# gusanagy/Hybrid-Diffusion-Underwater-Atmopheric-Image-Enhancement

Measured on AMD Instinct MI355X. Metric: denoising-steps/sec (256x256, T=1000), higher is better.
Workload: dtype f32 (tensors and accumulation fp32; every operand of the attention contractions as 2xfp16 pieces -- scores: a balance per product term, four terms at d_head 16 / three at d_head 32; P.V: three terms -- and of the 3x3 convs behind GroupNorm likewise (other 3x3 convs: 3xbf16 pieces), on the 16-bit MFM

## Files before the change

hybrid-diffusion-underwater-atmopheric-image-enhancement_amd/_capi.py:

```python
from __future__ import annotations

import ctypes as C
import os
import subprocess

_HERE = os.path.dirname(os.path.abspath(__file__))
LIB_PATH = os.environ.get("HDIFF_LIB", os.path.join(_HERE, "libhdiff.so"))
CSRC = os.path.join(_HERE, "csrc")
MAX_TAPS = 25

_lib = None


class LinearJob(C.Structure):
    _fields_ = [("w0", C.c_void_p), ("b0", C.c_void_p), ("w1", C.c_void_p), ("b1", C.c_void_p), ("y", C.c_void_p),
                ("n", C.c_int), ("first", C.c_int)]


class DdpmLoopDesc(C.Structure):
    _fields_ = [
        ("x", C.c_void_p), ("eps_c", C.c_void_p), ("eps_u", C.c_void_p), ("noise", C.c_void_p), ("x_next", C.c_void_p),
        ("coeff1", C.c_void_p), ("coeff2", C.c_void_p), ("sigma", C.c_void_p), ("step_ptr", C.c_void_p), ("T", C.c_int),
        ("w", C.c_double), ("seed", C.c_uint64), ("nan_flag", C.c_void_p), ("n", C.c_int64),
        ("x_dup0", C.c_void_p), ("x_dup1", C.c_void_p), ("t_next", C.c_void_p), ("t_count", C.c_int),
# ... 52 lines not shown
    ]


class WgradDesc(C.Structure):
    _fields_ = [
        ("x0", C.c_void_p), ("x1", C.c_void_p), ("C0", C.c_int), ("C1", C.c_int),
        ("B", C.c_int), ("H", C.c_int), ("W", C.c_int),
        ("gn_scale", C.c_void_p), ("gn_shift", C.c_void_p), ("dy", C.c_void_p),
        ("Cout", C.c_int), ("CinPad", C.c_int), ("CoutPad", C.c_int), ("OH", C.c_int), ("OW", C.c_int),
        ("VH", C.c_int), ("VW", C.c_int), ("in_stride", C.c_int),
        ("out_sy", C.c_int), ("out_oy", C.c_int), ("out_sx", C.c_int), ("out_ox", C.c_int),
        ("ntaps", C.c_int), ("tap_dy", C.c_int * MAX_TAPS), ("tap_dx", C.c_int * MAX_TAPS),
    ]


_PROTOS = {
    "hdiff_abi_version": (C.c_int, []),
    "hdiff_last_error": (C.c_char_p, []),
    "hdiff_device_count": (C.c_int, []),
    "hdiff_pack_conv_weight_x3": (C.c_int, [C.c_void_p, C.c_void_p, C.c_int, C.c_int, C.c_int, C.c_int, C.c_void_p]),
    "hdiff_pack_conv_weight_x3_taps": (C.c_int, [C.c_void_p, C.c_void_p, C.c_int, C.c_int, C.c_int, C.c_int, C.c_int, C.c_int,
                                                 C.POINTER(C.c_int), C.POINTER(C.c_int), C.c_int, C.c_void_p]),
    "hdiff_pack_conv_weight_h2_words": (C.c_int, [C.c_int, C.c_int, C.c_int, C.POINTER(C.c_int64)]),
    "hdiff_pack_conv_weight_h2": (C.c_int, [C.c_void_p, C.c_void_p, C.c_int, C.c_int, C.c_int, C.c_void_p]),
    "hdiff_gn_act_scale": (C.c_int, [C.c_void_p, C.c_void_p, C.c_int, C.c_int64, C.c_float, C.c_void_p, C.c_void_p]),
    "hdiff_set_contraction_mode": (C.c_int, [C.c_int]),
    "hdiff_get_contraction_mode": (C.c_int, []),
    "hdiff_pack_conv_weight": (C.c_int, [C.c_void_p, C.c_void_p, C.c_int, C.c_int, C.c_int, C.c_int, C.c_int, C.c_int,
                                         C.POINTER(C.c_int), C.POINTER(C.c_int), C.c_int, C.c_int, C.c_int, C.c_void_p]),
    "hdiff_conv2d_fwd": (C.c_int, [C.POINTER(ConvDesc), C.c_void_p]),
    "hdiff_conv2d_fwd_dropout": (C.c_int, [C.POINTER(ConvDesc), C.c_void_p, C.c_float, C.c_void_p]),
    "hdiff_conv2d_fwd_range": (C.c_int, [C.POINTER(ConvDesc), C.POINTER(ConvRange), C.c_void_p]),
    "hdiff_range_words_zero": (C.c_int, [C.c_void_p, C.c_int, C.c_void_p]),
    "hdiff_conv2d_fwd_route": (C.c_int, [C.POINTER(ConvDesc), C.POINTER(ConvRange), C.c_int, C.POINTER(C.c_int), C.POINTER(C.c_int)]),
    "hdiff_pack_conv_weight_h2_taps_words": (C.c_int, [C.c_int, C.c_int, C.c_int, C.c_int, C.POINTER(C.c_int64)]),
    "hdiff_pack_conv_weight_h2_taps": (C.c_int, [C.c_void_p, C.c_void_p, C.c_int, C.c_int, C.c_int, C.c_int, C.c_int, C.c_int,
                                                 C.POINTER(C.c_int), C.POINTER(C.c_int), C.c_int, C.c_void_p]),
    "hdiff_pack_conv_weight_h2_s2_words": (C.c_int, [C.c_int, C.c_int, C.c_int, C.POINTER(C.c_int64)]),
    "hdiff_pack_conv_weight_h2_s2": (C.c_int, [C.c_void_p, C.c_void_p, C.c_int, C.c_int, C.c_int, C.c_int, C.c_void_p]),
    "hdiff_conv2d_fwd_workspace": (C.c_int, [C.POINTER(ConvDesc), C.POINTER(C.c_int64)]),
    "hdiff_gn_stats": (C.c_int, [C.c_void_p, C.c_void_p, C.c_int, C.c_int, C.c_int, C.c_int, C.c_int, C.c_int, C.c_void_p,
                                 C.c_void_p]),
    "hdiff_gn_finalize": (C.c_int, [C.c_void_p, C.c_int, C.c_int, C.c_int, C.c_int, C.c_void_p, C.c_void_p, C.c_float,
                                    C.c_void_p, C.c_void_p, C.c_void_p, C.c_void_p, C.c_void_p]),
    "hdiff_gn_scale_shift": (C.c_int, [C.c_void_p, C.c_void_p, C.c_int, C.c_int, C.c_int, C.c_int, C.c_int, C.c_int, C.c_void_p,
                                       C.c_void_p, C.c_void_p, C.c_float, C.c_void_p, C.c_void_p, C.c_void_p]),
    "hdiff_gn_swish_apply": (C.c_int, [C.c_void_p, C.c_void_p, C.c_void_p, C.c_void_p, C.c_int, C.c_int, C.c_int,
                                       C.c_void_p]),
    "hdiff_mha_flash_fwd": (C.c_int, [C.c_void_p, C.c_void_p, C.c_void_p, C.c_int, C.c_int, C.c_int, C.c_int, C.c_void_p]),
    "hdiff_mha_flash_fwd_workspace": (C.c_int, [C.c_int, C.c_int, C.c_int, C.c_int, C.POINTER(C.c_int64)]),
    "hdiff_mha_flash_fwd_ws": (C.c_int, [C.c_void_p, C.c_void_p, C.c_void_p, C.c_int, C.c_int, C.c_int, C.c_int, C.c_void_p,
                                         C.c_int64, C.c_void_p]),
    "hdiff_mha_flash_fwd_route": (C.c_int, [C.c_int, C.c_int, C.c_int, C.c_int, C.c_int, C.c_int64] + [C.POINTER(C.c_int)] * 3),
    "hdiff_mha_wide_fwd": (C.c_int, [C.c_void_p, C.c_void_p, C.c_int, C.c_int, C.c_int, C.c_void_p]),
    "hdiff_mha_wide_bwd": (C.c_int, [C.c_void_p, C.c_void_p, C.c_void_p, C.c_void_p, C.c_int, C.c_int, C.c_int, C.c_void_p]),
    "hdiff_gn_affine_bwd": (C.c_int, [C.c_void_p, C.c_int, C.c_int, C.c_int, C.c_int, C.c_void_p, C.c_void_p, C.c_void_p, C.c_void_p,
                                      C.c_void_p, C.c_void_p, C.c_void_p, C.c_void_p, C.c_void_p, C.c_void_p]),
    "hdiff_gn_affine_apply": (C.c_int, [C.c_void_p, C.c_void_p, C.c_void_p, C.c_void_p, C.c_int, C.c_int, C.c_int,
                                        C.c_void_p]),
    "hdiff_mha_flash_bwd_workspace": (C.c_int, [C.c_int, C.c_int, C.c_int, C.c_int, C.POINTER(C.c_int64)]),
    "hdiff_mha_flash_bwd": (C.c_int, [C.c_void_p, C.c_void_p, C.c_void_p, C.c_void_p, C.c_void_p, C.c_void_p, C.c_void_p,
                                      C.c_int, C.c_int, C.c_int, C.c_int, C.c_void_p]),
    "hdiff_mha_flash_bwd_route": (C.c_int, [C.c_int, C.c_int, C.c_int, C.c_int] + [C.POINTER(C.c_int)] * 4),
    "hdiff_conv2d_wgrad_workspace": (C.c_int, [C.POINTER(WgradDesc), C.POINTER(C.c_int), C.POINTER(C.c_int64)]),
    "hdiff_conv2d_wgrad": (C.c_int, [C.POINTER(WgradDesc), C.c_void_p, C.c_int, C.c_void_p]),
    "hdiff_conv2d_wgrad_dropout": (C.c_int, [C.POINTER(WgradDesc), C.c_void_p, C.c_float, C.c_void_p, C.c_int, C.c_void_p]),
    "hdiff_conv2d_wgrad_route": (C.c_int, [C.POINTER(WgradDesc), C.c_int, C.POINTER(C.c_int)]),
    "hdiff_conv_wgrad_unpack": (C.c_int, [C.c_void_p, C.c_int, C.c_void_p, C.c_int, C.c_int, C.c_int, C.c_int, C.c_int, C.c_int,
                                          C.POINTER(C.c_int), C.POINTER(C.c_int), C.c_int, C.c_int, C.c_int, C.c_void_p]),
    "hdiff_gn_swish_bwd": (C.c_int, [C.c_void_p, C.c_void_p, C.c_int, C.c_int, C.c_int, C.c_int, C.c_int, C.c_void_p, C.c_void_p,
                                     C.c_void_p, C.c_void_p, C.c_void_p, C.c_void_p, C.c_void_p, C.c_void_p, C.c_void_p,
                                     C.c_void_p, C.c_void_p]),
    "hdiff_gn_swish_dropout_bwd": (C.c_int, [C.c_void_p, C.c_int, C.c_int, C.c_int, C.c_int, C.c_void_p, C.c_void_p, C.c_float,
                                             C.c_void_p, C.c_void_p, C.c_void_p, C.c_void_p, C.c_void_p, C.c_void_p, C.c_void_p,
                                             C.c_void_p, C.c_void_p]),
    "hdiff_bias_addvec_grad": (C.c_int, [C.c_void_p, C.c_int, C.c_int, C.c_int, C.c_void_p, C.c_void_p, C.c_void_p]),
    "hdiff_linear_rows_bwd": (C.c_int, [C.c_void_p, C.c_void_p, C.c_int, C.c_void_p, C.c_void_p, C.c_void_p, C.c_void_p,
                                        C.c_void_p, C.c_int, C.c_int, C.c_int, C.c_int, C.c_int, C.c_int, C.c_void_p]),
    "hdiff_sq_err_bwd": (C.c_int, [C.c_void_p, C.c_void_p, C.c_void_p, C.c_void_p, C.c_int64, C.c_void_p]),
    "hdiff_dropout_mask": (C.c_int, [C.c_void_p, C.c_int64, C.c_float, C.c_uint64, C.c_uint64, C.c_void_p]),
    "hdiff_dropout_keep_bits": (C.c_int, [C.c_void_p, C.c_int64, C.c_float, C.c_uint64, C.c_uint64, C.c_void_p]),
    "hdiff_mul": (C.c_int, [C.c_void_p, C.c_void_p, C.c_void_p, C.c_int64, C.c_void_p]),
    "hdiff_linear_rows": (C.c_int, [C.c_void_p, C.c_void_p, C.c_int, C.c_void_p, C.c_void_p, C.c_void_p, C.c_int, C.c_int,
                                    C.c_int, C.c_int, C.c_int, C.c_void_p]),
    "hdiff_linear_rows_multi": (C.c_int, [C.c_void_p, C.c_void_p, C.c_void_p, C.c_int, C.c_int, C.c_int, C.c_int, C.c_void_p]),
    "hdiff_q_sample": (C.c_int, [C.c_void_p, C.c_void_p, C.c_void_p, C.c_void_p, C.c_void_p, C.c_void_p, C.c_int, C.c_int,
                                 C.c_int, C.c_void_p]),
    "hdiff_sq_err": (C.c_int, [C.c_void_p, C.c_void_p, C.c_void_p, C.c_int64, C.c_void_p]),
    "hdiff_ddpm_step": (C.c_int, [C.c_void_p, C.c_void_p, C.c_void_p, C.c_void_p, C.c_void_p, C.c_void_p, C.c_void_p,
                                  C.c_void_p, C.c_void_p, C.c_int, C.c_double, C.c_uint64, C.c_void_p, C.c_int64, C.c_void_p]),
    "hdiff_ddpm_step_loop": (C.c_int, [C.c_void_p, C.c_void_p]),
    "hdiff_cfg_ddim_step": (C.c_int, [C.c_void_p, C.c_void_p, C.c_void_p, C.c_void_p, C.c_void_p, C.c_void_p, C.c_void_p, C.c_int,
                                      C.c_double, C.c_int, C.c_uint64, C.c_void_p, C.c_int64, C.c_void_p]),
    "hdiff_cfg_ddim_step_loop": (C.c_int, [C.c_void_p, C.c_void_p]),
    "hdiff_cfg_dpmpp_step": (C.c_int, [C.c_void_p, C.c_void_p, C.c_void_p, C.c_void_p, C.c_void_p, C.c_void_p, C.c_void_p, C.c_int,
                                       C.c_double, C.c_int, C.c_void_p, C.c_int64, C.c_void_p]),
    "hdiff_cfg_dpmpp_step_loop": (C.c_int, [C.c_void_p, C.c_void_p]),
    "hdiff_fill_t": (C.c_int, [C.c_void_p, C.c_void_p, C.c_int, C.c_void_p]),
    "hdiff_step_decrement": (C.c_int, [C.c_void_p, C.c_void_p]),
    "hdiff_ddim_step": (C.c_int, [C.c_void_p, C.c_void_p, C.c_void_p, C.c_void_p, C.c_void_p, C.c_int, C.c_void_p, C.c_int64,
                                  C.c_void_p]),
    "hdiff_fill_from_table": (C.c_int, [C.c_void_p, C.c_void_p, C.c_void_p, C.c_int, C.c_int, C.c_void_p]),
    "hdiff_tile_gather": (C.c_int, [C.c_void_p] * 4 + [C.c_int] * 10 + [C.c_void_p]),
    "hdiff_tile_ddim_step": (C.c_int, [C.c_void_p] * 12 + [C.c_int, C.c_void_p] + [C.c_int] * 8 + [C.c_void_p]),
    "hdiff_dpmpp_step": (C.c_int, [C.c_void_p] * 6 + [C.c_int, C.c_int, C.c_void_p, C.c_int64, C.c_void_p]),
    "hdiff_tile_dpmpp_step": (C.c_int, [C.c_void_p] * 13 + [C.c_int, C.c_int, C.c_void_p] + [C.c_int] * 8 + [C.c_void_p]),
# ... 146 lines not shown
```

hybrid-diffusion-underwater-atmopheric-image-enhancement_amd/csrc/attention.hip:

```cpp
#include <stdlib.h>

#include <type_traits>

#include "common.h"
#include "device.h"

using namespace hdiff;

namespace {

constexpr int KT = 64;
constexpr int KROW = KT + 4;
constexpr int ATT_THREADS = 256;
constexpr float RESCALE_LIMIT = 1.8446744e19f;

__device__ __forceinline__ f32x2 pk_add(f32x2 a, f32x2 b) {
  f32x2 r;
  asm("v_pk_add_f32 %0, %1, %2" : "=v"(r) : "v"(a), "v"(b));
  return r;
}

template <int D, int NQ>
__global__ __launch_bounds__(ATT_THREADS) void mha_flash_fwd_kernel(const float* __restrict__ qkv, float* __restrict__ out,
                                                                    float* __restrict__ lse2, int C, int L, float qscale, int check) {
// ... 384 lines not shown
  stage_load(0);
  stage_store(0);
  __syncthreads();
  stage_load(ntiles > 1 ? 1 : 0);
  do_tile(std::true_type{}, 0);
  stage_store(1);
  __syncthreads();
  auto step = [&](int t, auto buf_tag) {
    constexpr int buf = decltype(buf_tag)::value;
    stage_load((t + 1 < ntiles) ? t + 1 : t);
    do_tile(std::false_type{}, buf);
    stage_store(buf ^ 1);
    __syncthreads();
  };
  int t = 1;
  for (; t + 1 < ntiles; t += 2) {
    step(t, std::integral_constant<int, 1>{});
    step(t + 1, std::integral_constant<int, 0>{});
  }
  if (t < ntiles) step(t, std::integral_constant<int, 1>{});
  rowsum(NQ - 1);

  float* obase = out + ((size_t)b * C + (size_t)head * D) * L;
#pragma unroll
  for (int qt = 0; qt < NQ; ++qt) {
    float lt = l_run[qt].x + l_run[qt].y;
    lt += __shfl_xor(lt, 16, 64);
    lt += __shfl_xor(lt, 32, 64);
    const bool bad = !(lt < OVERFLOW_LIMIT);
    const float inv = bad ? __builtin_nanf("") : 1.0f / lt;
    const int q = qblk0 + qt * 16 + i16;
    if (lse2 != nullptr && q < L && g == 0)
      lse2[((size_t)b * gridDim.y + head) * L + q] = bad ? __builtin_nanf("") : __builtin_amdgcn_logf(lt) - negm4[qt][0];
    if (q < L) {
#pragma unroll
      for (int mt = 0; mt < MT; ++mt)
#pragma unroll
        for (int r = 0; r < 4; ++r) {
          const int d = mt * 16 + 4 * g + r;
          if (d < D) obase[(size_t)d * L + q] = O[mt][qt][r] * inv;
        }
    }
  }
}

template <int D, int NQ>
void launch_v(const float* qkv, float* o, float* lse2, int B, int C, int heads, int L, float qscale, int check,
              hipStream_t stream) {
  dim3 grid(cdiv(L, 64 * NQ), heads, B);
  hipLaunchKernelGGL((mha_flash_fwd_kernel<D, NQ>), grid, dim3(ATT_THREADS), 0, stream, qkv, o, lse2, C, L, qscale, check);
}

struct MhaFwdRoute { int route, nq, check; };
MhaFwdRoute mha_fwd_route(int B, int C, int heads, int L, bool want_lse, int64_t ws_bytes, int mode) {
  const int D = C / heads;
  if (D >= 48 || L < 512) return {HDIFF_MHA_FWD_ROUTE_RUNNING_MAX, 1, 0};
  if (mode != HDIFF_CONTRACT_F32) {
    const int64_t need = mha_fwd_x3p_workspace(B, C, heads, L);
    const bool ws_ok = need != 0 && ws_bytes >= need;
    if (mode == HDIFF_CONTRACT_F16 && !want_lse && ws_ok) return {HDIFF_MHA_FWD_ROUTE_F16_SINGLE, 4, 1};
    if (ws_ok && D == 16) return {HDIFF_MHA_FWD_ROUTE_H2_PAIRS, 4, 1};
    if (ws_ok && D == 32) return {HDIFF_MHA_FWD_ROUTE_X3P_PAIRS, 4, 1};
    if (L % KT == 0 && (D == 16 || D == 32)) return {HDIFF_MHA_FWD_ROUTE_X3_TRIPLES, 4, 1};
  }
  if (L % KT == 0) return {HDIFF_MHA_FWD_ROUTE_FAST_F32, 4, 1};
  return {HDIFF_MHA_FWD_ROUTE_RUNNING_MAX, 4, 0};
}

template <int D>
void launch_d(const float* qkv, float* o, float* lse2, int B, int C, int heads, int L, void* ws, const MhaFwdRoute& rt,
              hipStream_t stream) {
  const float qscale = 1.4426950408889634f / sqrtf((float)D);
  static const bool skip_check = getenv("HDIFF_NO_CHECK_PASS") != nullptr;
  const bool tail = !skip_check || rt.route == HDIFF_MHA_FWD_ROUTE_RUNNING_MAX || rt.route == HDIFF_MHA_FWD_ROUTE_FAST_F32;
  if constexpr (D < 48) {
    switch (rt.route) {
      case HDIFF_MHA_FWD_ROUTE_F16_SINGLE: launch_mha_fwd_f16(qkv, o, B, C, heads, L, qscale, ws, stream); break;
      case HDIFF_MHA_FWD_ROUTE_H2_PAIRS: launch_mha_fwd_h2(qkv, o, lse2, B, C, heads, L, qscale, ws, stream); break;
      case HDIFF_MHA_FWD_ROUTE_X3P_PAIRS: launch_mha_fwd_x3p(qkv, o, lse2, B, C, heads, L, qscale, ws, stream); break;
      case HDIFF_MHA_FWD_ROUTE_X3_TRIPLES: launch_mha_fwd_x3(qkv, o, lse2, B, C, heads, L, qscale, stream); break;
      case HDIFF_MHA_FWD_ROUTE_FAST_F32:
        hipLaunchKernelGGL((mha_flash_fwd_fast_kernel<D, 4>), dim3(cdiv(L, 256), heads, B), dim3(ATT_THREADS), 0, stream, qkv, o, lse2, C, L, qscale);
        break;
      default: break;
    }
    if (tail && rt.nq == 4) launch_v<D, 4>(qkv, o, lse2, B, C, heads, L, qscale, rt.check, stream);
  }
  if (tail && rt.nq == 1) launch_v<D, 1>(qkv, o, lse2, B, C, heads, L, qscale, rt.check, stream);
}

}

static int mha_fwd_check_shape(int B, int C, int heads, int L) {
  HDIFF_CHECK_ARG(B > 0 && L > 0 && heads > 0 && C % heads == 0, "mha_flash_fwd: bad sizes B=%d C=%d heads=%d L=%d", B, C,
                  heads, L);
  HDIFF_CHECK_ARG(mha_head_dim_ok(C / heads), "mha_flash_fwd: head dim %d not in {4, 8, 12, 16, 24, 32, 48, 64}", C / heads);
  return HDIFF_OK;
}

static int mha_flash_fwd_any(const float* qkv, float* o, float* lse2, int B, int C, int heads, int L, void* ws,
                             int64_t ws_bytes, hipStream_t s) {
  HDIFF_CHECK_ARG(qkv && o, "mha_flash_fwd: null pointer");
  const int rc = mha_fwd_check_shape(B, C, heads, L);
  if (rc != HDIFF_OK) return rc;
  const MhaFwdRoute rt = mha_fwd_route(B, C, heads, L, lse2 != nullptr, ws_bytes, contraction_mode());
  (void)hipGetLastError();
  with_head_dim(C / heads, [&](auto d) { launch_d<decltype(d)::value>(qkv, o, lse2, B, C, heads, L, ws, rt, s); });
  HDIFF_CHECK_LAUNCH("mha_flash_fwd_kernel");
  return HDIFF_OK;
}

extern "C" int hdiff_mha_flash_fwd(const float* qkv, float* o, float* lse2, int B, int C, int heads, int L,
                                   hdiff_stream_t stream) {
  return mha_flash_fwd_any(qkv, o, lse2, B, C, heads, L, nullptr, 0, (hipStream_t)stream);
}

extern "C" int hdiff_mha_flash_fwd_workspace(int B, int C, int heads, int L, int64_t* bytes_out) {
  HDIFF_CHECK_ARG(bytes_out, "mha_flash_fwd_workspace: null pointer");
  HDIFF_CHECK_ARG(B > 0 && L > 0 && heads > 0 && C % heads == 0, "mha_flash_fwd_workspace: bad sizes B=%d C=%d heads=%d L=%d", B,
                  C, heads, L);
  *bytes_out = mha_fwd_x3p_workspace(B, C, heads, L);
  return HDIFF_OK;
}

extern "C" int hdiff_mha_flash_fwd_ws(const float* qkv, float* o, float* lse2, int B, int C, int heads, int L, void* ws,
                                      int64_t ws_bytes, hdiff_stream_t stream) {
  HDIFF_CHECK_ARG(ws_bytes >= 0 && (ws != nullptr || ws_bytes == 0), "mha_flash_fwd_ws: workspace pointer / size mismatch");
  return mha_flash_fwd_any(qkv, o, lse2, B, C, heads, L, ws, ws_bytes, (hipStream_t)stream);
}

extern "C" int hdiff_mha_flash_fwd_route(int B, int C, int heads, int L, int want_lse, int64_t ws_bytes, int* route_out,
                                         int* nq_out, int* check_out) {
  HDIFF_CHECK_ARG(route_out && nq_out && check_out, "mha_flash_fwd_route: null pointer");
  HDIFF_CHECK_ARG(ws_bytes >= 0, "mha_flash_fwd_ws: workspace pointer / size mismatch");
  const int rc = mha_fwd_check_shape(B, C, heads, L);
  if (rc != HDIFF_OK) return rc;
  const MhaFwdRoute rt = mha_fwd_route(B, C, heads, L, want_lse != 0, ws_bytes, contraction_mode());
  *route_out = rt.route;
  *nq_out = rt.nq;
  *check_out = rt.check;
  return HDIFF_OK;
}
```

hybrid-diffusion-underwater-atmopheric-image-enhancement_amd/csrc/attention_h2.hip:

```cpp
#include <stdlib.h>

#include <type_traits>

#include "common.h"
#include "device.h"

using namespace hdiff;

namespace {

constexpr int KT = 64;
constexpr int THREADS = 256;
#define H2_RARE_BEGIN "s_cmp_lg_u64 %[cond], 0\n\ts_cbranch_scc1 .Lh2r_%=\n.Lh2b_%=:\n\t.subsection 1\n.Lh2r_%=:\n\t"
#define H2_RARE_END "s_branch .Lh2b_%=\n\t.subsection 0"

__device__ __forceinline__ float h2_rare_delta(unsigned long long cond, const f32x4 (&S)[4], int bp16, int bp32) {
  float delta, t, u;
  asm volatile(H2_RARE_BEGIN
               "v_max3_f32 %[t], %[s0], %[s1], %[s2]\n\t"
               "v_max3_f32 %[u], %[s3], %[s4], %[s5]\n\t"
               "v_max3_f32 %[t], %[t], %[s6], %[s7]\n\t"
               "v_max3_f32 %[u], %[u], %[s8], %[s9]\n\t"
               "v_max3_f32 %[t], %[t], %[s10], %[s11]\n\t"
               "v_max3_f32 %[u], %[u], %[s12], %[s13]\n\t"
// ... 92 lines not shown
  float mq = 0.f, mk = 0.f;
#pragma unroll
  for (int d = 0; d < D; ++d) {
    mq = fmaxf(mq, rowmax[(size_t)b * 2 * C + head * D + d]);
    mk = fmaxf(mk, rowmax[(size_t)b * 2 * C + C + head * D + d]);
  }
  const int a = balance_exp(__builtin_bit_cast(unsigned, mq), __builtin_bit_cast(unsigned, mk), qscale);
  const float sc = which == 0 ? qscale * __builtin_bit_cast(float, (unsigned)(127 - a) << 23) : __builtin_bit_cast(float, (unsigned)(127 + a) << 23);
  if (l >= L) return;
  const float* src = qkv + ((size_t)b * 3 * C + (size_t)which * C + (size_t)head * D) * L;
  const size_t piece = (size_t)L * D;
  __bf16* pair = ws + ((size_t)b * heads + head) * F_COUNT * piece;
  const float up = (float)(1 << PAIR_SHIFT) * one;
  unsigned h[4][D / 2];
#pragma unroll
  for (int j = 0; j < D / 2; ++j)
    pair4(src[(size_t)(2 * j) * L + l] * sc, src[(size_t)(2 * j + 1) * L + l] * sc, up, h[0][j], h[1][j], h[2][j], h[3][j]);
#pragma unroll
  for (int p = 0; p < 4; ++p) {
    if (which == 0 && (p == 1 || p == 3)) continue;
    const int slot = which == 0 ? F_Q + (p == 0 ? 0 : 1) : F_K + p;
    u32x4* o = reinterpret_cast<u32x4*>(pair + slot * piece + (size_t)l * D);
#pragma unroll
    for (int j = 0; j < D / 8; ++j) o[j] = u32x4{h[p][4 * j], h[p][4 * j + 1], h[p][4 * j + 2], h[p][4 * j + 3]};
  }
}

template <int D>
__global__ __launch_bounds__(THREADS) void v_split_h2_kernel(const float* __restrict__ qkv, __bf16* __restrict__ ws, int C, int L,
                                                             float one) {
  const int heads = C / D;
  const int row = blockIdx.x, head = row / D, d = row - head * D, b = blockIdx.y;
  const int tid = threadIdx.x;
  const float* src = qkv + ((size_t)b * 3 * C + 2 * (size_t)C + row) * L;
  const size_t piece = (size_t)L * D;
  __bf16* pair = ws + ((size_t)b * heads + head) * F_COUNT * piece;
  _Float16* dst = reinterpret_cast<_Float16*>(pair + F_V * piece) + (size_t)d * L;

  const float amax = row_absmax(src, L, tid);
  int e = (int)((__builtin_bit_cast(unsigned, amax) >> 23) & 0xffu) - 127;
  e = e < -100 ? -100 : (e > 127 ? 127 : e);
  const float scale = __builtin_bit_cast(float, (unsigned)(14 - e + 127) << 23);
  if (tid == 0) reinterpret_cast<float*>(pair + F_VINV * piece)[d] = __builtin_bit_cast(float, (unsigned)(e - 14 + 127) << 23);
  for (int i = tid; i < L / 4; i += THREADS) {
    const f32x4 v = *reinterpret_cast<const f32x4*>(src + 4 * (size_t)i);
    unsigned a0, a1, c0, c1;
    split2(v[0] * scale, v[1] * scale, one, a0, a1);
    split2(v[2] * scale, v[3] * scale, one, c0, c1);
    *reinterpret_cast<u32x2*>(dst + 4 * (size_t)i) = u32x2{a0, c0};
    *reinterpret_cast<u32x2*>(dst + piece + 4 * (size_t)i) = u32x2{a1, c1};
  }
}

template <int D, int NQ>
__global__ __launch_bounds__(THREADS, 2) void mha_flash_fwd_h2_kernel(const __bf16* __restrict__ ws, float* __restrict__ out,
                                                                      float* __restrict__ lse2, int C, int L, float one) {
  static_assert(D == 16, "head dim: two terms share one MFMA's 32 contraction slots");
  static_assert(NQ == 4, "the stage pipeline is written for four query tiles per wave");
  constexpr int NKP = 4;
  constexpr int NKS = 2;
  constexpr int NQK = NKS;
  constexpr int MT = D / 16;
  constexpr int KROWB = D * 2;
  constexpr int KPART = KT * KROWB;
  constexpr int VROWB = KT * 2 + 8;
  constexpr int VPART = D * VROWB;
  constexpr int QB = 64 * NQ;
  constexpr int VBASE = NKP * KPART;
  constexpr int BUFB = VBASE + 2 * VPART;
  __shared__ __attribute__((aligned(16))) unsigned char smem[2][BUFB];

  const int tid = threadIdx.x, lane = tid & 63, wave = tid >> 6;
  const int i16 = lane & 15, g = lane >> 4;
  const TileId tile = xcd_tile();
  const int head = tile.head, b = tile.b;
  const int qblk0 = tile.x * QB + wave * (16 * NQ);
  const int ntiles = L / KT;

  const int doff = 8 * (g & 1);
  const bool hi = g >> 1;

  const size_t piece_n = (size_t)L * D;
  const __bf16* wsq = ws + ((size_t)b * gridDim.y + head) * F_COUNT * piece_n;
  u32x4 qop[NQ][NQK];
  {
    const unsigned dn2 = PAIR_DOWN2;
#pragma unroll
    for (int qt = 0; qt < NQ; ++qt) {
      const int q = qblk0 + qt * 16 + i16;
      const u32x4 q0 = *reinterpret_cast<const u32x4*>(wsq + (size_t)q * D + doff);
      const u32x4 q1s = *reinterpret_cast<const u32x4*>(wsq + piece_n + (size_t)q * D + doff);
      const u32x4 sel = hi ? q1s : q0;
      unsigned dnw[4];
#pragma unroll
      for (int w = 0; w < 4; ++w) asm("v_pk_mul_f16 %0, %1, %2" : "=v"(dnw[w]) : "v"(sel[w]), "v"(dn2));
      qop[qt][0] = sel;
      qop[qt][1] = u32x4{dnw[0], dnw[1], dnw[2], dnw[3]};
    }
  }
  int kaddr[NKS];
#pragma unroll
  for (int ks = 0; ks < NKS; ++ks) kaddr[ks] = (2 * ks + (hi ? 1 : 0)) * KPART + i16 * KROWB + doff * 2;
  const int vaddr = i16 * VROWB + 8 * g;

  static_assert(2 * D * 8 == THREADS, "staging geometry: one V chunk per thread");
  static_assert(KPART == 2048 && THREADS == 256, "LDS-DMA geometry: eight 1 KiB runs, two per wave");
  const unsigned char* gsrc;
  int lds_off;
  u32x4 stage;
  {
    const __bf16* vsp = wsq + F_V * piece_n;
    const int p = tid / (D * 8), rem = tid - p * (D * 8);
    const int d = rem >> 3, seg = rem & 7;
    gsrc = reinterpret_cast<const unsigned char*>(vsp + p * piece_n + (size_t)d * L) + seg * 16;
    lds_off = VBASE + p * VPART + d * VROWB + seg * 16;
  }
  const unsigned lds0 = (unsigned)(size_t)(lds_byte*)&smem[0][0];
  const unsigned char* kdma = reinterpret_cast<const unsigned char*>(wsq + F_K * piece_n);
  auto dma_k = [&](int t, int buf) {
    const int ws_ = __builtin_amdgcn_readfirstlane(wave);
    const unsigned char* src = kdma + (size_t)ws_ * (piece_n * 2) + (size_t)t * KPART;
    const unsigned dst = __builtin_amdgcn_readfirstlane(lds0 + buf * BUFB + ws_ * KPART);
    dma_1k(src, lane * 16, dst);
    dma_1k(src + 1024, lane * 16, dst + 1024);
  };
  auto stage_load = [&](int t) { stage = *reinterpret_cast<const u32x4*>(gsrc + (size_t)t * (KT * 2)); };
  auto stage_store = [&](int buf) {
    unsigned char* dst = &smem[buf][lds_off];
    *reinterpret_cast<u32x2*>(dst) = u32x2{stage[0], stage[1]};
    *reinterpret_cast<u32x2*>(dst + 8) = u32x2{stage[2], stage[3]};
  };

  f32x4 O[MT][NQ];
  f32x4 negm4[NQ];
  float l_run[NQ];
  const int bp16 = (lane ^ 16) * 4, bp32 = (lane ^ 32) * 4;
#pragma unroll
  for (int qt = 0; qt < NQ; ++qt) {
    l_run[qt] = 0.f;
    negm4[qt] = f32x4{0.f, 0.f, 0.f, 0.f};
#pragma unroll
    for (int mt = 0; mt < MT; ++mt) O[mt][qt] = f32x4{0.f, 0.f, 0.f, 0.f};
// ... 93 lines not shown
        const int kt = n / 14, r = n - kt * 14;
        if (r < 4) pe[kt][r] = __builtin_amdgcn_exp2f(S[par][kt][r]);
        else if (r < 6) {
          const f16x2 p = {(_Float16)pe[kt][2 * (r - 4)], (_Float16)pe[kt][2 * (r - 4) + 1]};
          unsigned w = __builtin_bit_cast(unsigned, p);
          asm("" : "+v"(w));
          u[kt][r - 4] = w;
        } else if (r < 8) ad[kt][r - 6] = pe[kt][r - 6] + pe[kt][r - 6 + 2];
        else if (r < 10) rl[kt][r - 8] = (_Float16)__builtin_fmaf(pe[kt][2 * (r - 8)], one, -(float)__builtin_bit_cast(f16x2, u[kt][r - 8])[0]);
        else if (r < 12) {
          const f16x2 pr = {rl[kt][r - 10],
                            (_Float16)__builtin_fmaf(pe[kt][2 * (r - 10) + 1], one, -(float)__builtin_bit_cast(f16x2, u[kt][r - 10])[1])};
          unsigned w = __builtin_bit_cast(unsigned, pr);
          asm("" : "+v"(w));
          r2[kt][r - 10] = w;
        } else if (r == 12) sum0 = (kt == 0) ? ad[kt][0] : sum0 + ad[kt][0];
        else sum1 = (kt == 0) ? ad[kt][1] : sum1 + ad[kt][1];
      };
      constexpr int NV = 56;
#pragma unroll
      for (int i = 0; i < NM; ++i) {
        if constexpr (PEND) {
          const int npv = (i + 1) * NPV / NM, ppv = i * NPV / NM;
          if (npv != ppv) pv_mfma(pv_q, par ^ 1, ppv);
          else qk_mfma(qk_q, par ^ 1, i - ppv, rollk);
        } else qk_mfma(qk_q, par ^ 1, i, rollk);
#pragma unroll
        for (int n = NV * i / NM; n < NV * (i + 1) / NM; ++n) vstep(n);
        __builtin_amdgcn_sched_barrier(0);
      }
      const unsigned long long cond = __builtin_amdgcn_ballot_w64(sum0 + sum1 >= P_TRIP);
      const float delta = h2_rare_delta(cond, S[par], bp16, bp32);
      h2_rare_rescale(cond, delta, O[0][QT], negm4[QT], l_run[QT], sum0, sum1);
#pragma unroll
      for (int kt = 0; kt < 4; ++kt)
        h2_rare_exp_split(cond, delta, one, S[par][kt], u[kt][0], u[kt][1], r2[kt][0], r2[kt][1], sum0, sum1);
#pragma unroll
      for (int kt = 0; kt < 4; ++kt) {
        const int c = kt >> 1, o = (kt & 1) * 2;
        pop[par][0][c][o] = u[kt][0]; pop[par][1][c][o] = r2[kt][0];
        pop[par][0][c][o + 1] = u[kt][1]; pop[par][1][c][o + 1] = r2[kt][1];
      }
    }
    l_run[QT] += sum0 + sum1;
  };

  auto tile_fn = [&](auto first_tag, int t) {
    constexpr bool FIRST = decltype(first_tag)::value;
    using Pend = std::integral_constant<bool, !FIRST>;
    const int buf = t & 1;
    if constexpr (FIRST) load_v(buf);
    stage_fn(std::integral_constant<int, 0>{}, first_tag, Pend{});
    if constexpr (!FIRST) load_v(buf);
    stage_fn(std::integral_constant<int, 1>{}, first_tag, std::true_type{});
    stage_store(buf ^ 1);
    asm volatile("s_waitcnt vmcnt(0)" ::: "memory");
    __syncthreads();
    stage_load((t + 2 < ntiles) ? t + 2 : ntiles - 1);
    dma_k((t + 2 < ntiles) ? t + 2 : ntiles - 1, buf);
    stage_fn(std::integral_constant<int, 2>{}, first_tag, std::true_type{}, buf ^ 1);
    stage_fn(std::integral_constant<int, 3>{}, first_tag, std::true_type{});
  };

  stage_load(0);
  dma_k(0, 0);
  stage_store(0);
  asm volatile("s_waitcnt vmcnt(0)" ::: "memory");
  __syncthreads();
  stage_load(ntiles > 1 ? 1 : 0);
  dma_k(ntiles > 1 ? 1 : 0, 1);
  load_k(0);
#pragma unroll
  for (int n = 0; n < 4 * NQK; ++n) qk_mfma(0, 0, n);
  tile_fn(std::true_type{}, 0);
  for (int t = 1; t < ntiles; ++t) tile_fn(std::false_type{}, t);
#pragma unroll
  for (int n = 0; n < NPV; ++n) pv_mfma(NQ - 1, 1, n);

  float* obase = out + ((size_t)b * C + (size_t)head * D) * L;
  const float* vinv = reinterpret_cast<const float*>(wsq + F_VINV * piece_n);
#pragma unroll
  for (int qt = 0; qt < NQ; ++qt) {
    float lt = l_run[qt];
    lt += __shfl_xor(lt, 16, 64);
    lt += __shfl_xor(lt, 32, 64);
    const bool bad = !(lt < OVERFLOW_LIMIT);
    const float inv = bad ? __builtin_nanf("") : 1.0f / lt;
    const int q = qblk0 + qt * 16 + i16;
    if (lse2 != nullptr && g == 0)
      lse2[((size_t)b * gridDim.y + head) * L + q] = bad ? __builtin_nanf("") : __builtin_amdgcn_logf(lt) - negm4[qt][0];
#pragma unroll
    for (int mt = 0; mt < MT; ++mt)
#pragma unroll
      for (int r = 0; r < 4; ++r)
        obase[(size_t)(mt * 16 + 4 * g + r) * L + q] = (O[mt][qt][r] * inv) * vinv[mt * 16 + 4 * g + r];
  }
}

}

namespace hdiff {
void launch_v_split_h2(const float* qkv, void* ws, int B, int C, int heads, int L, hipStream_t stream) {
  if (C / heads == 16) hipLaunchKernelGGL((v_split_h2_kernel<16>), dim3(C, B), dim3(THREADS), 0, stream, qkv, (__bf16*)ws, C, L, 1.0f);
  else hipLaunchKernelGGL((v_split_h2_kernel<32>), dim3(C, B), dim3(THREADS), 0, stream, qkv, (__bf16*)ws, C, L, 1.0f);
}

int64_t mha_fwd_h2_tail_bytes(int B, int C) { return ((int64_t)B * 2 * C * 4 + 255) / 256 * 256; }

void launch_qk_split_h2(const float* qkv, void* ws, int B, int C, int heads, int L, float qscale, hipStream_t stream) {
  float* rowmax = reinterpret_cast<float*>(reinterpret_cast<unsigned char*>(ws) + mha_fwd_x3p_workspace(B, C, heads, L) - mha_fwd_h2_tail_bytes(B, C));
  hipLaunchKernelGGL(qk_rowmax_kernel, dim3(2 * C, B), dim3(THREADS), 0, stream, qkv, rowmax, C, L);
  dim3 grid(cdiv(L, 256), 2 * heads, B);
  if (C / heads == 16) hipLaunchKernelGGL((qk_split_h2_kernel<16>), grid, dim3(THREADS), 0, stream, qkv, rowmax, (__bf16*)ws, C, L, qscale, 1.0f);
  else hipLaunchKernelGGL((qk_split_h2_kernel<32>), grid, dim3(THREADS), 0, stream, qkv, rowmax, (__bf16*)ws, C, L, qscale, 1.0f);
}

void launch_mha_fwd_h2(const float* qkv, float* o, float* lse2, int B, int C, int heads, int L, float qscale, void* ws,
                       hipStream_t stream) {
  launch_qk_split_h2(qkv, ws, B, C, heads, L, qscale, stream);
  launch_v_split_h2(qkv, ws, B, C, heads, L, stream);
  hipLaunchKernelGGL((mha_flash_fwd_h2_kernel<16, 4>), dim3(L / 256, heads, B), dim3(THREADS), 0, stream, (const __bf16*)ws, o, lse2,
                     C, L, 1.0f);
}

}
```

hybrid-diffusion-underwater-atmopheric-image-enhancement_amd/csrc/common.h:

```cpp
#pragma once
#include <hip/hip_runtime.h>
#include <stdint.h>
#include <stdio.h>
#include <string.h>

#include <type_traits>

#include "../../include/hdiff.h"

namespace hdiff {

void set_error(const char* fmt, ...);

#define HDIFF_CHECK_ARG(cond, ...)            \
  do {                                        \
    if (!(cond)) {                            \
      hdiff::set_error(__VA_ARGS__);          \
      return HDIFF_ERR_INVALID;               \
    }                                         \
  } while (0)

#define HDIFF_CHECK_LAUNCH(what)                                                   \
  do {                                                                             \
    hipError_t e__ = hipGetLastError();                                            \
// ... 48 lines not shown

static inline bool first_use_on_device(uint64_t& mask) {
  int dev = 0;
  if (hipGetDevice(&dev) != hipSuccess || dev < 0 || dev >= 64) return true;
  const uint64_t bit = 1ull << dev;
  if (mask & bit) return false;
  mask |= bit;
  return true;
}

bool wgrad3x3_applicable(const hdiff_conv_wgrad_desc* d);
int wgrad3x3_nsplit(const hdiff_conv_wgrad_desc* d);
int launch_wgrad3x3(const hdiff_conv_wgrad_desc* d, float* dwp, int nsplit, hipStream_t stream, const unsigned* keep_bits = nullptr,
                    float inv_keep = 1.0f);
bool wgrad1x1_applicable(const hdiff_conv_wgrad_desc* d);
int wgrad1x1_nsplit(const hdiff_conv_wgrad_desc* d);
int launch_wgrad1x1(const hdiff_conv_wgrad_desc* d, float* dwp, int nsplit, hipStream_t stream);

int contraction_mode();
inline bool split_operands_on() { return contraction_mode() != HDIFF_CONTRACT_F32; }

static inline bool mha_head_dim_ok(int D) { return D == 4 || D == 8 || D == 12 || D == 16 || D == 24 || D == 32 || D == 48 || D == 64; }
template <class F>
static inline void with_head_dim(int D, F&& f) {
  switch (D) {
    case 4: return f(std::integral_constant<int, 4>{});
    case 8: return f(std::integral_constant<int, 8>{});
    case 12: return f(std::integral_constant<int, 12>{});
    case 16: return f(std::integral_constant<int, 16>{});
    case 24: return f(std::integral_constant<int, 24>{});
    case 32: return f(std::integral_constant<int, 32>{});
    case 48: return f(std::integral_constant<int, 48>{});
    case 64: return f(std::integral_constant<int, 64>{});
  }
}

struct KeyRanges { int per, nsplit; };
static inline KeyRanges key_ranges(int nkb_total, int want) {
  if (want > nkb_total) want = nkb_total;
  if (want < 1) want = 1;
  const int per = cdiv(nkb_total, want);
  return {per, cdiv(nkb_total, per)};
}
long long mha_bwd_slab_cap_bytes();
bool mha_bwd_x3_shape_ok(int B, int C, int heads, int L);
KeyRanges mha_bwd_h2_key_ranges(int B, int heads, int L, int D);
int64_t mha_bwd_x3_workspace_floats(int B, int C, int heads, int L);
bool mha_bwd_h2_lds_granted();
void launch_mha_bwd_h2(const float* qkv, const float* d_o, const float* lse2, const float* delta, float* dqkv, float* ws, int B,
                       int C, int heads, int L, KeyRanges g, hipStream_t stream);
int64_t mha_fwd_x3p_workspace(int B, int C, int heads, int L);
int64_t mha_fwd_h2_tail_bytes(int B, int C);
void launch_mha_fwd_x3p(const float* qkv, float* o, float* lse2, int B, int C, int heads, int L, float qscale, void* ws, hipStream_t stream);
void launch_mha_fwd_h2(const float* qkv, float* o, float* lse2, int B, int C, int heads, int L, float qscale, void* ws, hipStream_t stream);
void launch_qk_split_h2(const float* qkv, void* ws, int B, int C, int heads, int L, float qscale, hipStream_t stream);
void launch_v_split_h2(const float* qkv, void* ws, int B, int C, int heads, int L, hipStream_t stream);
void launch_mha_fwd_x3(const float* qkv, float* o, float* lse2, int B, int C, int heads, int L, float qscale, hipStream_t stream);
void launch_mha_fwd_f16(const float* qkv, float* o, int B, int C, int heads, int L, float qscale, void* ws, hipStream_t stream);

}
```

include/hdiff.h:

```cpp
#ifndef HDIFF_H_
#define HDIFF_H_

#include <stdint.h>

#ifdef __cplusplus
extern "C" {
#endif

typedef void* hdiff_stream_t;

enum hdiff_status {
  HDIFF_OK = 0,
  HDIFF_ERR_INVALID = -1,
  HDIFF_ERR_LAUNCH = -2,
  HDIFF_ERR_NO_DEVICE = -3
};

int hdiff_abi_version(void);
const char* hdiff_last_error(void);
int hdiff_device_count(void);
enum { HDIFF_CONTRACT_F32 = 0, HDIFF_CONTRACT_BF16X3 = 1, HDIFF_CONTRACT_F16 = 2 };
int hdiff_set_contraction_mode(int mode);
int hdiff_get_contraction_mode(void);

// ... 86 lines not shown
  int tap_dy[HDIFF_MAX_TAPS];
  int tap_dx[HDIFF_MAX_TAPS];
} hdiff_conv_wgrad_desc;
int hdiff_conv2d_wgrad_workspace(const hdiff_conv_wgrad_desc* d, int* nsplit_out, int64_t* floats_out);
int hdiff_conv2d_wgrad(const hdiff_conv_wgrad_desc* d, float* dwp, int nsplit, hdiff_stream_t stream);
int hdiff_conv2d_wgrad_dropout(const hdiff_conv_wgrad_desc* d, const uint32_t* keep_bits, float inv_keep, float* dwp, int nsplit,
                               hdiff_stream_t stream);
enum {
  HDIFF_WGRAD_ROUTE_FAST_1X1 = 0,
  HDIFF_WGRAD_ROUTE_FAST_3X3 = 1,
  HDIFF_WGRAD_ROUTE_GENERIC = 2,
  HDIFF_WGRAD_ROUTE_GENERIC_ROWS1 = 3,
  HDIFF_WGRAD_ROUTE_GENERIC_ROWS2 = 4
};
int hdiff_conv2d_wgrad_route(const hdiff_conv_wgrad_desc* d, int dropout, int* route_out);
int hdiff_conv_wgrad_unpack(const float* dwp, int nsplit, float* dw, int mode, int Cout, int Cin, int KH, int KW, int ntaps,
                            const int* tap_ky, const int* tap_kx, int CinPad, int CoutPad, int accumulate,
                            hdiff_stream_t stream);

int hdiff_gn_stats(const float* x0, const float* x1, int C0, int C1, int B, int HW, int G, int nsplit, float* ws,
                   hdiff_stream_t stream);
int hdiff_gn_finalize(const float* ws, int B, int C, int G, int nsplit, const float* gamma, const float* beta, float eps,
                      float* scale, float* shift, float* mean_out , float* rstd_out ,
                      hdiff_stream_t stream);
int hdiff_gn_scale_shift(const float* x0, const float* x1, int C0, int C1, int B, int HW, int G, int nsplit, float* ws,
                         const float* gamma, const float* beta, float eps, float* scale, float* shift,
                         hdiff_stream_t stream);
int hdiff_gn_swish_bwd(const float* x0, const float* x1, int C0, int C1, int B, int HW, int G, const float* dA,
                       const float* mean, const float* rstd, const float* gamma, const float* beta, float* ws, float* dx0,
                       float* dx1, float* dgamma, float* dbeta, hdiff_stream_t stream);
int hdiff_gn_swish_dropout_bwd(const float* x, int C, int B, int HW, int G, const float* dA, const uint32_t* keep_bits,
                               float inv_keep, const float* mean, const float* rstd, const float* gamma, const float* beta,
                               float* ws, float* dx, float* dgamma, float* dbeta, hdiff_stream_t stream);
int hdiff_gn_affine_bwd(const float* x, int C, int B, int HW, int G, const float* dY, const float* mean, const float* rstd,
                        const float* gamma, const float* beta, float* ws, float* dx, float* dgamma, float* dbeta,
                        hdiff_stream_t stream);
int hdiff_bias_addvec_grad(const float* dy, int B, int C, int HW, float* dvec, float* dbias, hdiff_stream_t stream);
int hdiff_gn_affine_apply(const float* x, const float* scale, const float* shift, float* y, int B, int C, int HW,
                          hdiff_stream_t stream);
int hdiff_gn_swish_apply(const float* x, const float* scale, const float* shift, float* y, int B, int C, int HW,
                         hdiff_stream_t stream);

int hdiff_mha_flash_fwd(const float* qkv, float* o, float* lse2 , int B, int C, int heads, int L,
                        hdiff_stream_t stream);
int hdiff_mha_flash_fwd_workspace(int B, int C, int heads, int L, int64_t* bytes_out);
int hdiff_mha_flash_fwd_ws(const float* qkv, float* o, float* lse2 , int B, int C, int heads, int L,
                           void* ws, int64_t ws_bytes, hdiff_stream_t stream);
enum {
  HDIFF_MHA_FWD_ROUTE_RUNNING_MAX = 0,
  HDIFF_MHA_FWD_ROUTE_FAST_F32 = 1,
  HDIFF_MHA_FWD_ROUTE_X3_TRIPLES = 2,
  HDIFF_MHA_FWD_ROUTE_H2_PAIRS = 3,
  HDIFF_MHA_FWD_ROUTE_X3P_PAIRS = 4,
  HDIFF_MHA_FWD_ROUTE_F16_SINGLE = 5
};
int hdiff_mha_flash_fwd_route(int B, int C, int heads, int L, int want_lse, int64_t ws_bytes, int* route_out, int* nq_out,
                              int* check_out);
int hdiff_mha_wide_fwd(const float* qkv, float* o, int B, int C, int L, hdiff_stream_t stream);
int hdiff_mha_wide_bwd(const float* qkv, const float* d_o, float* dqkv, float* ws, int B, int C, int L, hdiff_stream_t stream);
int hdiff_mha_flash_bwd_workspace(int B, int C, int heads, int L, int64_t* n_floats);
int hdiff_mha_flash_bwd(const float* qkv, const float* o, const float* d_o, const float* lse2, float* delta, float* dqkv,
                        float* ws, int B, int C, int heads, int L, hdiff_stream_t stream);
enum {
  HDIFF_MHA_BWD_ROUTE_FUSED_F32 = 0,
  HDIFF_MHA_BWD_ROUTE_H2_PAIRS = 1
};
int hdiff_mha_flash_bwd_route(int B, int C, int heads, int L, int* route_out, int* nk_out, int* aligned_out, int* nsplit_out);

int hdiff_linear_rows(const float* x, const int64_t* idx, int n_rows, const float* W, const float* bias, float* y, int B,
                      int K, int N, int swish_input, int accumulate, hdiff_stream_t stream);
typedef struct hdiff_linear_job {
  const float* w0; const float* b0; const float* w1; const float* b1; float* y;
  int n; int first;
} hdiff_linear_job;
int hdiff_linear_rows_multi(const float* x0 , const float* x1 , const hdiff_linear_job* jobs,
                            int njobs, int total_n, int B, int K, hdiff_stream_t stream);

int hdiff_linear_rows_bwd(const float* x, const int64_t* idx, int n_rows, const float* W, const float* dy, float* dx,
                          float* dW, float* db, int B, int K, int N, int swish_input, int accumulate, int pad_row,
                          hdiff_stream_t stream);

int hdiff_q_sample(const float* x0, const float* noise, const int64_t* t, const float* sqrt_ab, const float* sqrt_1mab,
                   float* xt, int B, int per_sample, int T, hdiff_stream_t stream);
int hdiff_sq_err(const float* a, const float* b, float* out, int64_t n, hdiff_stream_t stream);
int hdiff_sq_err_bwd(const float* a, const float* b, const float* dloss, float* da, int64_t n, hdiff_stream_t stream);
int hdiff_ddpm_step(const float* x, const float* eps_c, const float* eps_u, const float* noise, float* x_next,
                    const float* coeff1, const float* coeff2, const float* sigma, const int32_t* step_ptr,
                    int T , double w,
                    uint64_t seed, int32_t* nan_flag, int64_t n, hdiff_stream_t stream);
typedef struct hdiff_ddpm_loop_desc {
  const float* x; const float* eps_c; const float* eps_u;
  const float* noise;
  float* x_next;
  const float* coeff1; const float* coeff2; const float* sigma;
  int32_t* step_ptr;
  int T;
  double w;
  uint64_t seed;
  int32_t* nan_flag;
  int64_t n;
  float* x_dup0; float* x_dup1;
  int64_t* t_next; int t_count;
  uint32_t* done_counter;
} hdiff_ddpm_loop_desc;
int hdiff_ddpm_step_loop(const hdiff_ddpm_loop_desc* d, hdiff_stream_t stream);
int hdiff_cfg_ddim_step(const float* x, const float* eps_c, const float* eps_u, const float* noise, float* x_next,
                        const float* tab , const int32_t* step_ptr, int nsteps, double w, int clip_x0,
                        uint64_t seed, int32_t* nan_flag, int64_t n, hdiff_stream_t stream);
typedef struct hdiff_cfg_ddim_loop_desc {
  const float* x; const float* eps_c; const float* eps_u;
// ... 197 lines not shown
```

Before: 3.011.

## Add six-query-tile H2 attention variant chosen by wave-quantization cost model

Generalizes the H2 pairs flash-attention forward kernel to any even number of query tiles per wave, handling ragged tails, and adds a 384-query-block variant. A route heuristic compares estimated workgroup rounds over 512 slots for 256 and 384 query blocks and picks the larger block when it is cheaper, the aim being less wave-quantization tail and more K/V reuse per load. A new API entry lets callers force either H2 form. The cost is higher register and LDS pressure per workgroup and some wasted work on partial blocks.

```diff
diff --git a/hybrid-diffusion-underwater-atmopheric-image-enhancement_amd/_capi.py b/hybrid-diffusion-underwater-atmopheric-image-enhancement_amd/_capi.py
--- a/hybrid-diffusion-underwater-atmopheric-image-enhancement_amd/_capi.py
+++ b/hybrid-diffusion-underwater-atmopheric-image-enhancement_amd/_capi.py
@@ -128,6 +128,8 @@
     "hdiff_mha_flash_fwd_ws": (C.c_int, [C.c_void_p, C.c_void_p, C.c_void_p, C.c_int, C.c_int, C.c_int, C.c_int, C.c_void_p,
                                          C.c_int64, C.c_void_p]),
     "hdiff_mha_flash_fwd_route": (C.c_int, [C.c_int, C.c_int, C.c_int, C.c_int, C.c_int, C.c_int64] + [C.POINTER(C.c_int)] * 3),
+    "hdiff_mha_flash_fwd_ws_as": (C.c_int, [C.c_void_p, C.c_void_p, C.c_void_p, C.c_int, C.c_int, C.c_int, C.c_int, C.c_void_p,
+                                            C.c_int64, C.c_int, C.c_void_p]),
     "hdiff_mha_wide_fwd": (C.c_int, [C.c_void_p, C.c_void_p, C.c_int, C.c_int, C.c_int, C.c_void_p]),
     "hdiff_mha_wide_bwd": (C.c_int, [C.c_void_p, C.c_void_p, C.c_void_p, C.c_void_p, C.c_int, C.c_int, C.c_int, C.c_void_p]),
     "hdiff_gn_affine_bwd": (C.c_int, [C.c_void_p, C.c_int, C.c_int, C.c_int, C.c_int, C.c_void_p, C.c_void_p, C.c_void_p, C.c_void_p,
diff --git a/hybrid-diffusion-underwater-atmopheric-image-enhancement_amd/csrc/attention.hip b/hybrid-diffusion-underwater-atmopheric-image-enhancement_amd/csrc/attention.hip
--- a/hybrid-diffusion-underwater-atmopheric-image-enhancement_amd/csrc/attention.hip
+++ b/hybrid-diffusion-underwater-atmopheric-image-enhancement_amd/csrc/attention.hip
@@ -460,6 +460,15 @@
 }
 
 struct MhaFwdRoute { int route, nq, check; };
+
+constexpr int H2_WG_SLOTS = 2 * 256;
+constexpr double H2_Q384_G = 0.963;
+bool h2_q384_cheaper(int B, int heads, int L) {
+  const int64_t pairs = (int64_t)B * heads;
+  const int64_t r256 = (pairs * cdiv(L, 256) + H2_WG_SLOTS - 1) / H2_WG_SLOTS, r384 = (pairs * cdiv(L, 384) + H2_WG_SLOTS - 1) / H2_WG_SLOTS;
+  return H2_Q384_G * (double)(r384 * 384) < (double)(r256 * 256);
+}
+
 MhaFwdRoute mha_fwd_route(int B, int C, int heads, int L, bool want_lse, int64_t ws_bytes, int mode) {
   const int D = C / heads;
   if (D >= 48 || L < 512) return {HDIFF_MHA_FWD_ROUTE_RUNNING_MAX, 1, 0};
@@ -467,7 +476,7 @@
     const int64_t need = mha_fwd_x3p_workspace(B, C, heads, L);
     const bool ws_ok = need != 0 && ws_bytes >= need;
     if (mode == HDIFF_CONTRACT_F16 && !want_lse && ws_ok) return {HDIFF_MHA_FWD_ROUTE_F16_SINGLE, 4, 1};
-    if (ws_ok && D == 16) return {HDIFF_MHA_FWD_ROUTE_H2_PAIRS, 4, 1};
+    if (ws_ok && D == 16) return {h2_q384_cheaper(B, heads, L) ? HDIFF_MHA_FWD_ROUTE_H2_PAIRS_Q384 : HDIFF_MHA_FWD_ROUTE_H2_PAIRS, 4, 1};
     if (ws_ok && D == 32) return {HDIFF_MHA_FWD_ROUTE_X3P_PAIRS, 4, 1};
     if (L % KT == 0 && (D == 16 || D == 32)) return {HDIFF_MHA_FWD_ROUTE_X3_TRIPLES, 4, 1};
   }
@@ -484,7 +493,8 @@
   if constexpr (D < 48) {
     switch (rt.route) {
       case HDIFF_MHA_FWD_ROUTE_F16_SINGLE: launch_mha_fwd_f16(qkv, o, B, C, heads, L, qscale, ws, stream); break;
-      case HDIFF_MHA_FWD_ROUTE_H2_PAIRS: launch_mha_fwd_h2(qkv, o, lse2, B, C, heads, L, qscale, ws, stream); break;
+      case HDIFF_MHA_FWD_ROUTE_H2_PAIRS: launch_mha_fwd_h2(qkv, o, lse2, B, C, heads, L, qscale, ws, 4, stream); break;
+      case HDIFF_MHA_FWD_ROUTE_H2_PAIRS_Q384: launch_mha_fwd_h2(qkv, o, lse2, B, C, heads, L, qscale, ws, 6, stream); break;
       case HDIFF_MHA_FWD_ROUTE_X3P_PAIRS: launch_mha_fwd_x3p(qkv, o, lse2, B, C, heads, L, qscale, ws, stream); break;
       case HDIFF_MHA_FWD_ROUTE_X3_TRIPLES: launch_mha_fwd_x3(qkv, o, lse2, B, C, heads, L, qscale, stream); break;
       case HDIFF_MHA_FWD_ROUTE_FAST_F32:
@@ -507,11 +517,16 @@
 }
 
 static int mha_flash_fwd_any(const float* qkv, float* o, float* lse2, int B, int C, int heads, int L, void* ws,
-                             int64_t ws_bytes, hipStream_t s) {
+                             int64_t ws_bytes, hipStream_t s, int as_route = -1) {
   HDIFF_CHECK_ARG(qkv && o, "mha_flash_fwd: null pointer");
   const int rc = mha_fwd_check_shape(B, C, heads, L);
   if (rc != HDIFF_OK) return rc;
-  const MhaFwdRoute rt = mha_fwd_route(B, C, heads, L, lse2 != nullptr, ws_bytes, contraction_mode());
+  MhaFwdRoute rt = mha_fwd_route(B, C, heads, L, lse2 != nullptr, ws_bytes, contraction_mode());
+  if (as_route >= 0 && as_route != rt.route) {
+    auto h2 = [](int r) { return r == HDIFF_MHA_FWD_ROUTE_H2_PAIRS || r == HDIFF_MHA_FWD_ROUTE_H2_PAIRS_Q384; };
+    HDIFF_CHECK_ARG(h2(as_route) && h2(rt.route), "mha_flash_fwd_ws_as: route %d is no form of this call's route %d", as_route, rt.route);
+    rt.route = as_route;
+  }
   (void)hipGetLastError();
   with_head_dim(C / heads, [&](auto d) { launch_d<decltype(d)::value>(qkv, o, lse2, B, C, heads, L, ws, rt, s); });
   HDIFF_CHECK_LAUNCH("mha_flash_fwd_kernel");
@@ -535,6 +550,13 @@
                                       int64_t ws_bytes, hdiff_stream_t stream) {
   HDIFF_CHECK_ARG(ws_bytes >= 0 && (ws != nullptr || ws_bytes == 0), "mha_flash_fwd_ws: workspace pointer / size mismatch");
   return mha_flash_fwd_any(qkv, o, lse2, B, C, heads, L, ws, ws_bytes, (hipStream_t)stream);
+}
+
+extern "C" int hdiff_mha_flash_fwd_ws_as(const float* qkv, float* o, float* lse2, int B, int C, int heads, int L, void* ws,
+                                         int64_t ws_bytes, int route, hdiff_stream_t stream) {
+  HDIFF_CHECK_ARG(ws_bytes >= 0 && (ws != nullptr || ws_bytes == 0), "mha_flash_fwd_ws: workspace pointer / size mismatch");
+  HDIFF_CHECK_ARG(route >= 0, "mha_flash_fwd_ws_as: route %d", route);
+  return mha_flash_fwd_any(qkv, o, lse2, B, C, heads, L, ws, ws_bytes, (hipStream_t)stream, route);
 }
 
 extern "C" int hdiff_mha_flash_fwd_route(int B, int C, int heads, int L, int want_lse, int64_t ws_bytes, int* route_out,
diff --git a/hybrid-diffusion-underwater-atmopheric-image-enhancement_amd/csrc/attention_h2.hip b/hybrid-diffusion-underwater-atmopheric-image-enhancement_amd/csrc/attention_h2.hip
--- a/hybrid-diffusion-underwater-atmopheric-image-enhancement_amd/csrc/attention_h2.hip
+++ b/hybrid-diffusion-underwater-atmopheric-image-enhancement_amd/csrc/attention_h2.hip
@@ -168,11 +168,19 @@
   }
 }
 
+template <int FROM, int TO, class F>
+__device__ __forceinline__ void static_for(F&& f) {
+  if constexpr (FROM < TO) {
+    f(std::integral_constant<int, FROM>{});
+    static_for<FROM + 1, TO>(f);
+  }
+}
+
 template <int D, int NQ>
 __global__ __launch_bounds__(THREADS, 2) void mha_flash_fwd_h2_kernel(const __bf16* __restrict__ ws, float* __restrict__ out,
                                                                       float* __restrict__ lse2, int C, int L, float one) {
   static_assert(D == 16, "head dim: two terms share one MFMA's 32 contraction slots");
-  static_assert(NQ == 4, "the stage pipeline is written for four query tiles per wave");
+  static_assert(NQ >= 4 && (NQ & 1) == 0, "the S / P double buffers alternate by the query tile's parity: an even number of tiles per wave");
   constexpr int NKP = 4;
   constexpr int NKS = 2;
   constexpr int NQK = NKS;
@@ -182,6 +190,7 @@
   constexpr int VROWB = KT * 2 + 8;
   constexpr int VPART = D * VROWB;
   constexpr int QB = 64 * NQ;
+  constexpr bool RAGGED = 256 % QB != 0;
   constexpr int VBASE = NKP * KPART;
   constexpr int BUFB = VBASE + 2 * VPART;
   __shared__ __attribute__((aligned(16))) unsigned char smem[2][BUFB];
@@ -203,7 +212,8 @@
     const unsigned dn2 = PAIR_DOWN2;
 #pragma unroll
     for (int qt = 0; qt < NQ; ++qt) {
-      const int q = qblk0 + qt * 16 + i16;
+      const int qt0 = qblk0 + qt * 16;
+      const int q = (RAGGED && qt0 >= L ? 0 : qt0) + i16;
       const u32x4 q0 = *reinterpret_cast<const u32x4*>(wsq + (size_t)q * D + doff);
       const u32x4 q1s = *reinterpret_cast<const u32x4*>(wsq + piece_n + (size_t)q * D + doff);
       const u32x4 sel = hi ? q1s : q0;
@@ -403,14 +413,18 @@
     if constexpr (FIRST) load_v(buf);
     stage_fn(std::integral_constant<int, 0>{}, first_tag, Pend{});
     if constexpr (!FIRST) load_v(buf);
-    stage_fn(std::integral_constant<int, 1>{}, first_tag, std::true_type{});
-    stage_store(buf ^ 1);
-    asm volatile("s_waitcnt vmcnt(0)" ::: "memory");
-    __syncthreads();
-    stage_load((t + 2 < ntiles) ? t + 2 : ntiles - 1);
-    dma_k((t + 2 < ntiles) ? t + 2 : ntiles - 1, buf);
-    stage_fn(std::integral_constant<int, 2>{}, first_tag, std::true_type{}, buf ^ 1);
-    stage_fn(std::integral_constant<int, 3>{}, first_tag, std::true_type{});
+    static_for<1, NQ>([&](auto qt_tag) {
+      constexpr int QT = decltype(qt_tag)::value;
+      if constexpr (QT == NQ - 2) stage_fn(qt_tag, first_tag, std::true_type{}, buf ^ 1);
+      else stage_fn(qt_tag, first_tag, std::true_type{});
+      if constexpr (QT == NQ / 2 - 1) {
+        stage_store(buf ^ 1);
+        asm volatile("s_waitcnt vmcnt(0)" ::: "memory");
+        __syncthreads();
+        stage_load((t + 2 < ntiles) ? t + 2 : ntiles - 1);
+        dma_k((t + 2 < ntiles) ? t + 2 : ntiles - 1, buf);
+      }
+    });
   };
 
   stage_load(0);
@@ -438,6 +452,7 @@
     const bool bad = !(lt < OVERFLOW_LIMIT);
     const float inv = bad ? __builtin_nanf("") : 1.0f / lt;
     const int q = qblk0 + qt * 16 + i16;
+    if (RAGGED && qblk0 + qt * 16 >= L) continue;
     if (lse2 != nullptr && g == 0)
       lse2[((size_t)b * gridDim.y + head) * L + q] = bad ? __builtin_nanf("") : __builtin_amdgcn_logf(lt) - negm4[qt][0];
 #pragma unroll
@@ -466,12 +481,15 @@
   else hipLaunchKernelGGL((qk_split_h2_kernel<32>), grid, dim3(THREADS), 0, stream, qkv, rowmax, (__bf16*)ws, C, L, qscale, 1.0f);
 }
 
-void launch_mha_fwd_h2(const float* qkv, float* o, float* lse2, int B, int C, int heads, int L, float qscale, void* ws,
+void launch_mha_fwd_h2(const float* qkv, float* o, float* lse2, int B, int C, int heads, int L, float qscale, void* ws, int nq,
                        hipStream_t stream) {
   launch_qk_split_h2(qkv, ws, B, C, heads, L, qscale, stream);
   launch_v_split_h2(qkv, ws, B, C, heads, L, stream);
-  hipLaunchKernelGGL((mha_flash_fwd_h2_kernel<16, 4>), dim3(L / 256, heads, B), dim3(THREADS), 0, stream, (const __bf16*)ws, o, lse2,
-                     C, L, 1.0f);
-}
-
-}
+  const dim3 grid(cdiv(L, 64 * nq), heads, B);
+  if (nq == 6)
+    hipLaunchKernelGGL((mha_flash_fwd_h2_kernel<16, 6>), grid, dim3(THREADS), 0, stream, (const __bf16*)ws, o, lse2, C, L, 1.0f);
+  else
+    hipLaunchKernelGGL((mha_flash_fwd_h2_kernel<16, 4>), grid, dim3(THREADS), 0, stream, (const __bf16*)ws, o, lse2, C, L, 1.0f);
+}
+
+}
diff --git a/hybrid-diffusion-underwater-atmopheric-image-enhancement_amd/csrc/common.h b/hybrid-diffusion-underwater-atmopheric-image-enhancement_amd/csrc/common.h
--- a/hybrid-diffusion-underwater-atmopheric-image-enhancement_amd/csrc/common.h
+++ b/hybrid-diffusion-underwater-atmopheric-image-enhancement_amd/csrc/common.h
@@ -124,7 +124,8 @@
 int64_t mha_fwd_x3p_workspace(int B, int C, int heads, int L);
 int64_t mha_fwd_h2_tail_bytes(int B, int C);
 void launch_mha_fwd_x3p(const float* qkv, float* o, float* lse2, int B, int C, int heads, int L, float qscale, void* ws, hipStream_t stream);
-void launch_mha_fwd_h2(const float* qkv, float* o, float* lse2, int B, int C, int heads, int L, float qscale, void* ws, hipStream_t stream);
+void launch_mha_fwd_h2(const float* qkv, float* o, float* lse2, int B, int C, int heads, int L, float qscale, void* ws, int nq,
+                       hipStream_t stream);
 void launch_qk_split_h2(const float* qkv, void* ws, int B, int C, int heads, int L, float qscale, hipStream_t stream);
 void launch_v_split_h2(const float* qkv, void* ws, int B, int C, int heads, int L, hipStream_t stream);
 void launch_mha_fwd_x3(const float* qkv, float* o, float* lse2, int B, int C, int heads, int L, float qscale, hipStream_t stream);
diff --git a/include/hdiff.h b/include/hdiff.h
--- a/include/hdiff.h
+++ b/include/hdiff.h
@@ -162,10 +162,13 @@
   HDIFF_MHA_FWD_ROUTE_X3_TRIPLES = 2,
   HDIFF_MHA_FWD_ROUTE_H2_PAIRS = 3,
   HDIFF_MHA_FWD_ROUTE_X3P_PAIRS = 4,
-  HDIFF_MHA_FWD_ROUTE_F16_SINGLE = 5
+  HDIFF_MHA_FWD_ROUTE_F16_SINGLE = 5,
+  HDIFF_MHA_FWD_ROUTE_H2_PAIRS_Q384
 };
 int hdiff_mha_flash_fwd_route(int B, int C, int heads, int L, int want_lse, int64_t ws_bytes, int* route_out, int* nq_out,
                               int* check_out);
+int hdiff_mha_flash_fwd_ws_as(const float* qkv, float* o, float* lse2 , int B, int C, int heads, int L,
+                              void* ws, int64_t ws_bytes, int route, hdiff_stream_t stream);
 int hdiff_mha_wide_fwd(const float* qkv, float* o, int B, int C, int L, hdiff_stream_t stream);
 int hdiff_mha_wide_bwd(const float* qkv, const float* d_o, float* dqkv, float* ws, int B, int C, int L, hdiff_stream_t stream);
 int hdiff_mha_flash_bwd_workspace(int B, int C, int heads, int L, int64_t* n_floats);
```

Result: faster. 3.084 (median of 6 runs) (+2.4%).
